# tangrizzly/Point-of-Interest-Recommendation

Measured on AMD Instinct MI355X. Metric: check-in sequences/sec training (Distance2Pre) + all-POI top-K eval users/sec, higher is better.
Workload: dtype f32 (forward pass: int8 x 5 fixed point + f64 gates); 1 GPU; synthetic gowalla-shape: 100000 POIs, 50000 users, seq<=50, dim=128, 200 distance bins; one step = one Distance2Pre training epoch over all users; batch_rule=capped sum, cap 64, parallelism=user-shard x1, per-epoch delta all-reduce, table_storage=f32

## Files before the change

### point-of-interest-recommendation_amd/csrc/abi.hip

```cpp
#include "../../include/poi_hip.h"
#include "poi_kernels.h"

#include <math.h>
#include <stdarg.h>
#include <stdio.h>
#include <stdlib.h>
#include <string.h>
#include <string>
#include <utility>
#include <vector>

namespace {
thread_local std::string g_err;
}

struct DevBuf {
  void* p = nullptr;
  size_t bytes = 0;
};

struct poi_ctx {
  int device = 0;
  int num_cu = 0;
  int wg_per_cu = 2;
  std::string err;
  DevBuf ws, slab, te_ws, hslab, zrow;
  DevBuf ex_ws, ex_slab, ex_glt, ex_gdi;
  int engine = 0;
  float batch_cap = 1.0f;
  int wgrad_rounds = 2;
  int head_rounds = 3;
  int score_variant = -1;
  DevBuf g_lt, mult_lt, nseq_lt, g_di, mult_di, nseq_di;
  DevBuf g_wd, mult_wd, nseq_wd, ca_ws, ca_slab, ca_scr, ca2;
  int carnn_fast = 1;
  hipEvent_t ev_hr0 = nullptr, ev_hr1 = nullptr;
  int hot_early = 1;
  hipStream_t side2 = nullptr; hipEvent_t ev_h0 = nullptr, ev_h1 = nullptr, ev_h2 = nullptr, ev_h3 = nullptr;
  int hybrid = 1, hyb_min = 1150, hyb_max = 2300, hyb_force = 0;
  hipStream_t side = nullptr; hipEvent_t ev_slots = nullptr, ev_sorted = nullptr, ev_bwd = nullptr, ev_fin = nullptr, ev_start = nullptr, ev_pack = nullptr;
  DevBuf seg_s, seg_e;
  DevBuf xc;
  DevBuf pmark;
  int ppoi = 1;
  int hot_bins = 1;
  int early_bins = 1;
  int early_min = 1024;
  DevBuf kc_dev;
  DevBuf ptab, iota;
  int iota_n = -1;
  int fwd_tab = 1;
  int bintab_min = 1280;
  int one_path = 1;
// ... 208 lines not shown
  ++c->te_ws_gen;
  const int n_dist = spatial ? P->n_dist : -1;
  const int D = P->dim, NBP = poi::te_nbp(n_dist);
  A.lt = P->lt; A.di = P->di; A.ui = P->ui; A.wh = P->wh; A.bi = P->bi; A.vs = P->vs; A.bs = P->bs; A.wd = P->wd; A.lw = P->lw;
  A.n_item = P->n_item; A.n_dist = n_dist; A.dim = D;
  A.spatial = spatial ? 1 : 0; A.xw = spatial ? 2 * D : D;
  A.lt_f16 = is_f16(c, P->lt);
  A.bintab = (poi::te_bintab(D, spatial, n_dist) && (predict || n >= c->bintab_min)) ? 1 : 0;
  A.rec32 = (D >= 256 || (D == 128 && c->engine == 3)) ? 1 : 0;
  A.rec_split = c->rec_split ? 1 : 0;
  A.head_split = (c->rec_split && A.spatial && (P->n_dist + 1 > 256 || (c->head3 && !predict))) ? 1 : 0;
  A.efuse = (c->efuse && A.head_split && !predict && P->n_dist + 1 <= 256 && D == 128) ? 1 : 0;
  A.rec1 = (!A.rec32 && n <= c->rec1_max) ? 1 : 0;
  A.hyb = (c->hybrid && c->side2 && !predict && !A.rec32 && D == 128 && c->xfwd && poi::te_xfwd_supported(D) && c->rec_split && n >= c->hyb_min && n <= c->hyb_max && n <= TE_HYB_NMAX && n > 1) ? 1 : 0;
  A.hyb_force = c->hyb_force;
  if (A.hyb) A.rec1 = 0;
  A.ppoi = (A.bintab && !predict && c->ppoi) ? 1 : 0;
  A.off = T->off; A.p = T->p; A.q = T->q; A.dp = T->dp; A.dq = T->dq; A.len_max = T->len_max;
  A.uidx = uidx; A.n_seq = n; A.predict = predict ? 1 : 0;
  if (const char* e = getenv("POI_TE_DBG")) A.dbg = atoi(e);
  A.dl = poi::dense_layout(D, A.xw, n_dist + 1);
  const size_t Tcap = (size_t)n * (size_t)(predict ? T->max_len : (T->max_len > 1 ? T->max_len - 1 : 1)) + 192;
  const size_t pk = (size_t)30 * D * D + (size_t)3 * NBP * D + 128;
  const bool sorted = !predict;
  const size_t Ncap = sorted ? 3 * (Tcap + (size_t)n) : 0;
  const size_t n_hot = Ncap / (TE_COLD_MAX + 1) + 2, n_chunk = Ncap / TE_HOT_CHUNK + n_hot + 2;
  const size_t sfl = sorted ? Tcap + n_chunk * D + Tcap * (size_t)NBP + (size_t)((n <= c->rec1_max || n <= c->hyb_max) ? n : (n + 15) / 16) * 3 * D + (size_t)2 * ((n + 255) / 256) + 128 : 0;
  const int Rrows = P->n_item + 1 + n_dist + 1;
  const bool listed = sorted && (size_t)Rrows > 4 * Ncap;
  const size_t sin = sorted ? 7 * Ncap + (listed ? Ncap : 0) + (size_t)RS_HIST_INTS + RS_MAXBIN + 16 + 4 * n_hot + 3 * n_chunk + 64 : 0;
// ... 55 lines not shown
  A.pVsT = (float4*)take((size_t)NBP * D * 3 / 2); A.pVs = (float4*)take((size_t)NBP * D * 3 / 2);
  A.pWhT16 = (float4*)take((size_t)9 * D * D / 2); A.pWhc16 = (float4*)take((size_t)3 * D * D / 2); A.pWhzr16 = (float4*)take((size_t)3 * D * D);
  if (A.hyb) { A.pWhc1 = (float4*)take((size_t)D * D); A.pWhzr1 = (float4*)take((size_t)2 * D * D); } else { A.pWhc1 = A.pWhc16; A.pWhzr1 = A.pWhzr16; }
  if (A.bintab) {
    A.ztab = take(NBt * 3 * D); A.dsum = take(NBt * 3 * D); A.dgd = take(NBt * D);
    if (sorted) { A.dpart = take(n_dchunk * (size_t)(3 * D)); A.dpart2 = take(n_dsuper * (size_t)(3 * D)); }
  }
  if (A.ppoi) { A.S = take(Tcap * (size_t)(3 * D)); A.pfirst = take(n_prange * (size_t)(3 * D)); A.plast = take(n_prange * (size_t)(3 * D)); }
  if (sorted) {
    A.gcoef = take(Tcap); A.hot_part = take(n_chunk * D); A.DL = take(Tcap * (size_t)NBP);
    A.bi_part = take((size_t)((A.rec1 || A.hyb) ? n : (n + 15) / 16) * 3 * D); A.fin_part = take((size_t)2 * ((n + 255) / 256) + 8);
  }
  int* ip = (int*)f;
  auto itake = [&](size_t cnt) { int* r = ip; ip += (cnt + 3) & ~(size_t)3; return r; };
  A.hyb_dev = itake(8);
  A.soff = itake(n + 1); A.row_src = itake(Tcap); A.row_t = itake(Tcap); A.row_p = itake(Tcap); A.row_dp = itake(Tcap); A.row_ab = itake(Tcap); A.row_pq = (int2*)itake(2 * Tcap);
  if (sorted) {
    int bits = 1; while ((1 << bits) <= R) ++bits;
    A.key_bits = bits;
    A.keys0 = itake(Ncap); A.keys1 = itake(Ncap); A.vals0 = itake(Ncap); A.vals1 = itake(Ncap);
    A.code = itake(Ncap); A.slot_seq = itake(Ncap); A.ent = itake(Ncap);
    A.hist = itake(RS_HIST_INTS + RS_MAXBIN);
    A.cnt = itake(8);
    A.urow = listed ? itake(Ncap) : nullptr;
    A.hot_rows = (int4*)itake(4 * n_hot); A.hot_chunks = (int2*)itake(2 * n_chunk); A.hot_nf = itake(n_chunk);
    A.seg_start = (int*)c->seg_s.p; A.seg_end = (int*)c->seg_e.p;
    A.dch0 = itake(NBt + 8); A.dhot = itake(NBt + 16); A.dcc0 = itake(NBt + 8);
    if (A.ppoi) {
      A.urow_p = itake(Tcap); A.pblk = itake(2 * 1024); A.dxe = itake(Tcap); A.dxs = itake(Tcap); A.dstart = itake(Tcap + 4);
      A.pmark = (int*)c->pmark.p;
// ... 1519 lines not shown
}

int poi_ctx_set_exact_forward(poi_ctx* c, int on, int per_sequence_max) {
  if (!c || on < 0 || on > 1) return fail(c, POI_EINVAL, "poi_ctx_set_exact_forward: on must be 0 or 1");
  c->xfwd = on;
  if (per_sequence_max >= 0) c->xrec1_max = per_sequence_max;
  drop_graphs(c);
  return POI_OK;
}

int poi_ctx_set_option(poi_ctx* c, const char* name, int value) {
  if (!c || !name) return fail(c, POI_EINVAL, "poi_ctx_set_option: null argument");
  struct Opt { const char* name; int* p; int lo, hi; };
  const Opt opts[] = {{"forward_table_compact", &c->xcomp, 0, 1}, {"forward_table_compact_min", &c->xcomp_min, 0, 1 << 30}, {"head_split", &c->head3, 0, 1},
                      {"early_bins", &c->early_bins, 0, 1}, {"hot_bins", &c->hot_bins, 0, 1}, {"hybrid", &c->hybrid, 0, 1}, {"hybrid_min", &c->hyb_min, 0, 1 << 30}, {"hybrid_max", &c->hyb_max, 0, 1 << 30}, {"hybrid_force", &c->hyb_force, 0, 1 << 30},
                      {"cell_grid", &c->cell_grid, 0, 1 << 30}, {"vbpr_grid", &c->vbpr_grid, 0, 1 << 30}, {"session_tile_min", &c->sess_tile_min, 1, 1 << 30},
                      {"near_split_max", &c->near_split_max, 0, 1 << 30}, {"near_grid", &c->near_grid, 0, NEAR_SPLIT_LIMIT},
                      {"rank_grid", &c->rank_grid, 0, 1 << 30}};
  for (const Opt& o : opts)
    if (!strcmp(name, o.name)) {
      if (value < o.lo || value > o.hi) return fail(c, POI_EINVAL, "poi_ctx_set_option: %s must be in [%d, %d] (got %d)", name, o.lo, o.hi, value);
      *o.p = value;
      drop_graphs(c);
      return POI_OK;
    }
  return fail(c, POI_EINVAL, "poi_ctx_set_option: unknown option '%s'", name);
}

int poi_ctx_set_small_launch(poi_ctx* c, int max_sequences) {
  if (!c || max_sequences < 0) return fail(c, POI_EINVAL, "poi_ctx_set_small_launch: max_sequences must be >= 0");
// ... 163 lines not shown
```

### point-of-interest-recommendation_amd/csrc/poi_common.h

```cpp
#pragma once
#include <hip/hip_runtime.h>
#include <mutex>
#include <hip/hip_fp16.h>
#include <stdint.h>

#define POI_WAVE 64
#define POI_BLOCK 256
#define POI_NWAVE (POI_BLOCK / POI_WAVE)

namespace poi {

__device__ __forceinline__ int lane_id() { return threadIdx.x & 63; }
__device__ __forceinline__ int wave_id() { return threadIdx.x >> 6; }

template <int CTRL>
__device__ __forceinline__ float dpp_f(float v) {
  return __int_as_float(__builtin_amdgcn_update_dpp(0, __float_as_int(v), CTRL, 0xF, 0xF, false));
}
__device__ __forceinline__ float readlane_f(float v, int l) {
  return __int_as_float(__builtin_amdgcn_readlane(__float_as_int(v), l));
}

__device__ __forceinline__ float wave_sum(float v) {
  v += dpp_f<0xB1>(v);
  v += dpp_f<0x4E>(v);
  v += dpp_f<0x141>(v);
  v += dpp_f<0x140>(v);
  return (readlane_f(v, 0) + readlane_f(v, 16)) + (readlane_f(v, 32) + readlane_f(v, 48));
// ... 222 lines not shown
struct DeviceOnce {
  std::mutex mu;
  bool done[64] = {};
  template <class F> hipError_t run(F&& f) {
    int dev = 0;
    hipError_t e = hipGetDevice(&dev);
    if (e != hipSuccess) return e;
    if (dev < 0 || dev >= 64) return hipErrorInvalidDevice;
    std::lock_guard<std::mutex> lock(mu);
    if (done[dev]) return hipSuccess;
    e = f();
    if (e == hipSuccess) done[dev] = true;
    return e;
  }
};
}
```

### point-of-interest-recommendation_amd/csrc/poi_kernels.h

```cpp
#pragma once
#include <hip/hip_runtime.h>
#include <stddef.h>
#include <stdint.h>

#include <string>
#include <vector>

namespace poi {

struct Timing {
  struct Rec { std::string name; hipEvent_t a, b; };
  bool on = false;
  int period = 1; unsigned long count = 0; bool active = true;
  void tick() { active = period <= 1 || (count++ % (unsigned long)period) == 0; }
  std::vector<Rec> recs;
  size_t limit = 32768;
  void begin(const char* name, hipStream_t st) {
    if (!on || !active || recs.size() >= limit) { open_ = false; return; }
    Rec r; r.name = name;
    if (hipEventCreate(&r.a) != hipSuccess || hipEventCreate(&r.b) != hipSuccess) { open_ = false; return; }
    (void)hipEventRecord(r.a, st);
    recs.push_back(r); open_ = true;
  }
  void end(hipStream_t st) { if (open_) { (void)hipEventRecord(recs.back().b, st); open_ = false; } }
// ... 89 lines not shown
  float* ptab; const int* iota; int fwd_tab; float* uiP;
  float4* pUiP3;
  float* uiT;
  float4 *pWhT16, *pWhc16, *pWhzr16;
  int rec_split;
  int head_split;
  int rec1;
  float* slab;
  int n_slab, n_head, n_kc;
  hipStream_t side; hipEvent_t ev_slots, ev_sorted;
  hipEvent_t ev_start, ev_pack;
  hipEvent_t ev_bwd, ev_fin;
  int hot_early; hipEvent_t ev_hr0, ev_hr1;
  int hyb, hyb_force; int* hyb_dev; float4 *pWhc1, *pWhzr1;
  hipStream_t side2; hipEvent_t ev_h0, ev_h1, ev_h2, ev_h3;
  float *bi_part, *fin_part;
  float* hslab; int hstride;
  DenseLayout dl;
  int *mult_lt, *nseq_lt, *mult_di, *nseq_di;
  float *hts, *sts; const int* out_row;
  int key_bits;
  int *keys0, *keys1, *vals0, *vals1;
  int *code, *slot_seq;
  int *ent;
  int *seg_start, *seg_end;
  int *hist;
  int *cnt;
  int *urow;
  int4* hot_rows;
  int2* hot_chunks;
// ... 458 lines not shown
```

### point-of-interest-recommendation_amd/csrc/te_xfwd.hip

```cpp
#include "poi_common.h"
#include "poi_kernels.h"

#include <stdio.h>
#include <type_traits>

namespace poi {

typedef int i32x4 __attribute__((ext_vector_type(4)));
typedef int i32x16 __attribute__((ext_vector_type(16)));

#define XS 5
#define XQB (8 * XS - 2)

__device__ __forceinline__ void x_lds_barrier() {
  asm volatile("s_waitcnt lgkmcnt(0)" ::: "memory");
  __builtin_amdgcn_s_barrier();
  asm volatile("" ::: "memory");
}
__device__ __forceinline__ double x_pow2(int e) { return __longlong_as_double((long long)(1023 + e) << 52); }
__device__ __forceinline__ int x_exponent(float m) { return (int)((__float_as_uint(m) >> 23) & 255u) - 126; }

__device__ __forceinline__ void x_digits(double t, unsigned& lo, unsigned& hi) {
  const unsigned long long b = (unsigned long long)__double_as_longlong(t + 0x1.8p52) + 0x8080808080ull;
  lo = (unsigned)b ^ 0x80808080u;
// ... 248 lines not shown
#else
#define XP_INIT
#define XP(i)
#define XP_END
#endif
struct XG12 { double v[12]; };

template <int D, bool FT, bool PRED = false>
__global__ __launch_bounds__(D * 4) void te_rec_fwdx_kernel(TeArgs A) {
  constexpr int KB = D / 64, NW = D / 16, SR = 3, SL = XS - SR, LDP = D + 16, PSZ = 16 * LDP;
  static_assert(D <= 128 && D % 64 == 0, "te_rec_fwdx: resident digit fragments and x_combine's int32 merge are sized for K <= 128");
  extern __shared__ __align__(16) unsigned char xlds[];
  unsigned char* Hq = xlds;
  unsigned char* RHq = Hq + XS * PSZ;
  uint4* Bl = reinterpret_cast<uint4*>(RHq + XS * PSZ) + (size_t)wave_id() * (3 * KB * SL * 64);
  __shared__ int s_r0[16], s_ns[16];
  __shared__ double s_t64[64];
  __shared__ __align__(16) double s_cn[3 * D];
  const int lane = lane_id(), w = wave_id(), tid = threadIdx.x, i = lane & 15;
  const int u0 = 16 * w + 4 * (lane >> 4);
  const int tile = blockIdx.x;
  const int k_lo = (!PRED && A.hyb) ? A.hyb_dev[0] : 0;
  if (k_lo + tile * 16 >= A.n_seq) return;
  if (tid < 16) {
    const int k = k_lo + tile * 16 + tid;
    int r0 = 0, ns = 0;
    if (k < A.n_seq) { r0 = A.soff[k]; ns = A.soff[k + 1] - r0; }
    s_r0[tid] = r0; s_ns[tid] = ns;
  }
  if (tid >= 64 && tid < 128) s_t64[tid - 64] = exp2((double)(tid - 64) * (1.0 / 64.0));
  for (int e = tid; e < 3 * D; e += blockDim.x) s_cn[e] = A.xWhS[e] * 0x1p-8;
  for (int e = tid; e < 2 * XS * PSZ / 4; e += blockDim.x) reinterpret_cast<unsigned*>(xlds)[e] = 0u;
  i32x4 bw[3][KB][SR];
#pragma unroll
  for (int gt = 0; gt < 3; ++gt) {
    const int nt = gt * NW + w;
#pragma unroll
    for (int kb = 0; kb < KB; ++kb)
#pragma unroll
      for (int s = 0; s < XS; ++s) {
        const uint4 v = A.xWh8[((size_t)(nt * KB + kb) * XS + s) * 64 + lane];
        if (s < SR) bw[gt][kb][s] = __builtin_bit_cast(i32x4, v);
        else Bl[((gt * KB + kb) * SL + (s - SR)) * 64 + lane] = v;
      }
  }
  __syncthreads();
  int ns_max = 0;
  for (int q = 0; q < 16; ++q) ns_max = max(ns_max, s_ns[q]);
  const int rowb = s_r0[i], nsr = s_ns[i];
  const int Tsp = A.soff[A.n_seq];
  const double h_init = (A.xflag && *A.xflag == A.xlaunch) ? __longlong_as_double(0x7FF8000000000000ll) : 0.0;
  double hcur[4] = {h_init, h_init, h_init, h_init};
  XG12 gc;
  struct XG4 { double v[4]; };
  auto load3 = [&](XG12& o, const double* __restrict__ rowp) {
#pragma unroll
    for (int g = 0; g < 3; ++g) {
      const XG4 q = *reinterpret_cast<const XG4*>(rowp + g * D + u0);
#pragma unroll
      for (int r = 0; r < 4; ++r) o.v[4 * g + r] = q.v[r];
    }
  };
  XP_INIT

  const unsigned char* hrow = Hq + i * LDP + 16 * (lane >> 4);
  const unsigned char* rrow = RHq + i * LDP + 16 * (lane >> 4);
  auto put_digits = [&](unsigned char* plane0, const double (&v)[4]) {
    unsigned lo[4], hi[4];
#pragma unroll
    for (int r = 0; r < 4; ++r) x_digits38(v[r], lo[r], hi[r]);
    unsigned* at = reinterpret_cast<unsigned*>(plane0 + i * LDP + u0);
    at[0] = x_gather_byte(hi[0], hi[1], hi[2], hi[3], 0);
#pragma unroll
    for (int s = 1; s < XS; ++s) at[s * (PSZ / 4)] = x_gather_byte(lo[0], lo[1], lo[2], lo[3], XS - 1 - s);
  };
  auto mma = [&](auto& acc, const unsigned char* __restrict__ h0, const int gt0, auto ng) {
    constexpr int NG = decltype(ng)::value;
#pragma unroll
    for (int g = 0; g < NG; ++g)
// ... 71 lines not shown
    auto fetch = [&](int t, XG12& n) { load3(n, A.gx + (size_t)(t < nsr ? rowb + t : Tsp) * 3 * D); };
    XG12 nx;
    fetch(0, gc);
    for (int t = 0; t < ns_max; ++t) {
      fetch(t + 1, nx);
      compute(t);
#pragma unroll
      for (int q = 0; q < 12; ++q) {
        asm volatile("" : "+v"(nx.v[q]));
        gc.v[q] = nx.v[q];
      }
    }
  } else {
    int rp = 0, rz = 0;
    const int* __restrict__ xrow = A.xcomp ? A.row_pc : A.row_p;
    auto ids = [&](int t) { const int rr = t < nsr ? rowb + t : Tsp; rp = xrow[rr]; rz = A.spatial ? A.row_dp[rr] : 0; };
    auto rows = [&](XG12& pp, XG12& zz) {
      const int p1 = (int)min((unsigned)rp, (unsigned)A.n_item), z1 = A.spatial ? (int)min((unsigned)rz, (unsigned)A.n_dist) : 0;
      load3(pp, A.ptabx + (size_t)p1 * 3 * D);
      load3(zz, A.ztabx + (size_t)z1 * 3 * D);
    };
    XG12 pn, zn;
    ids(0); rows(pn, zn);
#pragma unroll
    for (int q = 0; q < 12; ++q) gc.v[q] = pn.v[q] + zn.v[q];
    ids(1);
    for (int t = 0; t < ns_max; ++t) {
      rows(pn, zn);
      ids(t + 2);
      compute(t);
#pragma unroll
      for (int q = 0; q < 12; ++q) {
        asm volatile("" : "+v"(pn.v[q]), "+v"(zn.v[q]));
        gc.v[q] = pn.v[q] + zn.v[q];
      }
    }
  }
  if constexpr (PRED) {
    const int k = tile * 16 + i;
    if (k < A.n_seq)
      *reinterpret_cast<float4*>(A.hts + (size_t)(A.out_row ? A.out_row[k] : k) * D + u0) = make_float4((float)hcur[0], (float)hcur[1], (float)hcur[2], (float)hcur[3]);
  }
  XP_END
}

template <int CTRL>
__device__ __forceinline__ double x_dpp(double v) {
  const long long b = __double_as_longlong(v);
  const int lo = __builtin_amdgcn_update_dpp(0, (int)b, CTRL, 0xF, 0xF, false), hi = __builtin_amdgcn_update_dpp(0, (int)(b >> 32), CTRL, 0xF, 0xF, false);
  return __longlong_as_double(((long long)hi << 32) | (unsigned)lo);
}
template <int N> __device__ __forceinline__ double x_group_sum(double v) {
  v += x_dpp<0xB1>(v);
  v += x_dpp<0x4E>(v);
  v += x_dpp<0x141>(v);
  if (N >= 16) v += x_dpp<0x140>(v);
// ... 262 lines not shown
size_t te_xfwd_lds(int D) {
  const int KB = D / 64, NW = D / 16, SL = XS - 3;
  return (size_t)2 * XS * 16 * (D + 16) + (size_t)NW * 3 * KB * SL * 64 * 16;
}

size_t te_xfrag_bytes(int rows, int K) { return (size_t)rows * K * XS; }

template <int D> struct XRec {
  static constexpr bool F64 = D > 128;
  static size_t lds() { return F64 ? sizeof(double) * 2 * D * 16 : te_xfwd_lds(D <= 128 ? D : 128); }
  static dim3 block() { return dim3(F64 ? D * 2 : D * 4); }
  template <bool FT, bool PRED> static const void* fn() {
    if constexpr (F64) return reinterpret_cast<const void*>(&te_rec_fwdd_kernel<D, FT, PRED>);
    else return reinterpret_cast<const void*>(&te_rec_fwdx_kernel<D, FT, PRED>);
  }
  template <bool FT, bool PRED> static void launch(const TeArgs& A, hipStream_t st) {
    const dim3 grid((A.n_seq + 15) / 16);
    if constexpr (F64) hipLaunchKernelGGL((te_rec_fwdd_kernel<D, FT, PRED>), grid, block(), lds(), st, A);
    else hipLaunchKernelGGL((te_rec_fwdx_kernel<D, FT, PRED>), grid, block(), lds(), st, A);
  }
};

template <int D>
static hipError_t te_xfwd_t(const TeArgs& A, int num_cu, hipStream_t st, Timing* tm, int phase) {
  static DeviceOnce once;
  {
    const hipError_t oe = once.run([&]() -> hipError_t {
      const void* fns[5] = {XRec<D>::template fn<false, false>(), XRec<D>::template fn<true, false>(), XRec<D>::template fn<false, true>(), XRec<D>::template fn<true, true>(),
                            reinterpret_cast<const void*>(&te_gemmx_kernel<D>)};
      for (const void* f : fns) {
        const hipError_t e = hipFuncSetAttribute(f, hipFuncAttributeMaxDynamicSharedMemorySize, 152 * 1024);
        if (e != hipSuccess) return e;
      }
      return hipSuccess;
// ... 58 lines not shown
      for (int i = 0; i < 8; ++i) fprintf(stderr, " %s %.1f%%;", nm[i], 100.0 * (double)h[w][i] / (double)tot);
      fprintf(stderr, "\n");
    }
    unsigned long long z[8][10] = {};
    (void)hipMemcpyToSymbol(HIP_SYMBOL(g_xprof), z, sizeof(z));
  } } dump_at_exit;
#endif
  if (A.predict) {
    if constexpr (!XRec<D>::F64) {
      if (A.xrec1) {
        if (A.xft) hipLaunchKernelGGL((te_rec_fwd1x_kernel<D, true, true>), dim3(min(n, num_cu * (D <= 64 ? 3 : 1))), dim3(4 * D), 0, st, A);
        else hipLaunchKernelGGL((te_rec_fwd1x_kernel<D, true, false>), dim3(min(n, num_cu * (D <= 64 ? 3 : 1))), dim3(4 * D), 0, st, A);
        return hipGetLastError();
      }
    }
    if (A.xft) XRec<D>::template launch<true, true>(A, st);
    else XRec<D>::template launch<false, true>(A, st);
    return hipGetLastError();
  }
  tm->begin("te_rec_fwd", st);
  bool done = false;
  if constexpr (!XRec<D>::F64) {
    if (A.hyb) {
      if (hipEventRecord(A.ev_h0, st) != hipSuccess || hipStreamWaitEvent(A.side2, A.ev_h0, 0) != hipSuccess) return hipGetLastError();
      if (A.xft) hipLaunchKernelGGL((te_rec_fwd1x_kernel<D, false, true>), dim3(min(n, num_cu)), dim3(4 * D), 0, A.side2, A);
      else hipLaunchKernelGGL((te_rec_fwd1x_kernel<D, false, false>), dim3(min(n, num_cu)), dim3(4 * D), 0, A.side2, A);
      if (hipEventRecord(A.ev_h1, A.side2) != hipSuccess) return hipGetLastError();
      if (A.xft) XRec<D>::template launch<true, false>(A, st);
      else XRec<D>::template launch<false, false>(A, st);
      if (hipStreamWaitEvent(st, A.ev_h1, 0) != hipSuccess) return hipGetLastError();
      done = true;
    } else
    if (A.xrec1) {
      if (A.xft) hipLaunchKernelGGL((te_rec_fwd1x_kernel<D, false, true>), dim3(min(n, num_cu * (D <= 64 ? 3 : 1))), dim3(4 * D), 0, st, A);
      else hipLaunchKernelGGL((te_rec_fwd1x_kernel<D, false, false>), dim3(min(n, num_cu * (D <= 64 ? 3 : 1))), dim3(4 * D), 0, st, A);
      done = true;
    }
  }
  if (!done) {
    if (A.xft) XRec<D>::template launch<true, false>(A, st);
    else XRec<D>::template launch<false, false>(A, st);
  }
  tm->end(st);
  return hipGetLastError();
}

hipError_t launch_te_xfwd(const TeArgs& A, int num_cu, hipStream_t st, Timing* tm, int phase) {
  if (A.dim == 64) return te_xfwd_t<64>(A, num_cu, st, tm, phase);
  if (A.dim == 128) return te_xfwd_t<128>(A, num_cu, st, tm, phase);
  if (A.dim == 256) return te_xfwd_t<256>(A, num_cu, st, tm, phase);
  return hipErrorInvalidValue;
}

}
```

### point-of-interest-recommendation_amd/csrc/tile_engine.hip

```cpp
#include "poi_common.h"
#include "poi_kernels.h"

#include <stdlib.h>
#include <stdio.h>

namespace poi {

typedef float f32x16 __attribute__((ext_vector_type(16)));

#define TE_BLOCK 256

__device__ __forceinline__ f32x16 mfma32(float a, float b, f32x16 c) {
  return __builtin_amdgcn_mfma_f32_32x32x2f32(a, b, c, 0, 0, 0);
}
__device__ __forceinline__ void lds_barrier() {
  asm volatile("s_waitcnt lgkmcnt(0)" ::: "memory");
  __builtin_amdgcn_s_barrier();
  asm volatile("" ::: "memory");
}
__device__ __forceinline__ float fast_tanh(float x) { return 1.0f - 2.0f * __builtin_amdgcn_rcpf(1.0f + __expf(2.0f * x)); }
__device__ __forceinline__ float fast_sigmoid(float x) { return __builtin_amdgcn_rcpf(1.0f + __expf(-x)); }
__device__ __forceinline__ int c_row(int r, int lane) { return (r & 3) + 8 * (r >> 2) + 4 * (lane >> 5); }

struct PackJob { const float* src; int sk, sn, K, N, K8, NT; float4* dst; int n16; };
// ... 475 lines not shown
#pragma unroll
      for (int o = 1; o < 16; o <<= 1) { const int t2 = __shfl_up(t, o, 64); t += lane >= o ? t2 : 0; }
      if (lane < 16) wtot[lane] = t;
    }
    __syncthreads();
    const int run = carry + inc - s + (w > 0 ? wtot[w - 1] : 0);
    if (base == 0) my_pre = run;
#pragma unroll
    for (int u = 0; u < 16; ++u) if (i0 + u < n) A.soff[i0 + u] = run + v[u];
    carry += wtot[15];
    __syncthreads();
  }
  if (tid == 1023) {
    const int total = carry;
    A.soff[n] = total;
    if (A.cnt) { A.cnt[0] = (A.spatial ? 3 : 2) * (total + n); A.cnt[1] = 0; A.cnt[2] = 0; A.cnt[3] = 0; A.cnt[4] = 0; A.cnt[5] = 0; }
  }
  if (A.hyb && n <= TE_HYB_NMAX) te_hybrid_choose(A, num_cu, my_max, my_pre, carry, s_hmax, s_hpre, s_hcost, s_harg, s_hlen);
}

#ifndef TE_SEQ_PER_WAVE
#define TE_SEQ_PER_WAVE 4
#endif
__device__ __forceinline__ void te_slots(const TeArgs& A, int k, int base, int L, int ns, int r0, int* pads_lt, int* pads_di) {
  const int lane = lane_id();
  const int nsec = A.spatial ? 3 : 2;
  const int S0 = nsec * (r0 + k), nslot = nsec * (ns + 1), sentinel = A.n_item + 1 + A.n_dist + 1;
  int plt = 0, pdi = 0;
  for (int e0 = 0; e0 < nslot; e0 += 64) {
    const int e = e0 + lane;
// ... 807 lines not shown
  sbz += __shfl_xor(sbz, 16, 64); sbr += __shfl_xor(sbr, 16, 64); sbc += __shfl_xor(sbc, 16, 64);
  sbz += __shfl_xor(sbz, 32, 64); sbr += __shfl_xor(sbr, 32, 64); sbc += __shfl_xor(sbc, 32, 64);
  if (lane < 16) {
    float* bp = A.bi_part + (size_t)tile * 3 * D;
    bp[col] = sbz; bp[D + col] = sbr; bp[2 * D + col] = sbc;
  }
}

template <int D>
__global__ __launch_bounds__(D * 4) void te_rec_bwd16t_kernel(TeArgs A) {
  extern __shared__ __align__(16) float lds[];
  constexpr int KG2 = D / 32, LHA = D + 8, LHB = 2 * D + 8;
  unsigned short* Acs = reinterpret_cast<unsigned short*>(lds);
  unsigned short* Azrs = Acs + 3 * 16 * LHA;
  uint4* B3 = reinterpret_cast<uint4*>(Azrs + 3 * 16 * LHB) + (size_t)wave_id() * 3 * KG2 * 64;
  __shared__ int s_r0[16], s_ns[16];
  const int lane = lane_id(), w = wave_id(), tid = threadIdx.x;
  const int sq = lane & 15, u0 = 16 * w + 4 * (lane >> 4);
  const int tile = blockIdx.x;
  const int k_lo = A.hyb ? A.hyb_dev[2] : 0;
  if (k_lo + tile * 16 >= A.n_seq) return;
  if (tid < 16) {
    const int k = k_lo + tile * 16 + tid;
    int r0 = 0, ns = 0;
    if (k < A.n_seq) { r0 = A.soff[k]; ns = A.soff[k + 1] - r0; }
    s_r0[tid] = r0; s_ns[tid] = ns;
  }
  lds_barrier();
  int ns_max = 0;
  for (int i = 0; i < 16; ++i) ns_max = max(ns_max, s_ns[i]);
  const int rowb = s_r0[sq], nsr = s_ns[sq];
  uint4 bcb[KG2][2], bzrb[2 * KG2][2];
  const uint4 *cc3 = B3 + lane, *czr3 = B3 + KG2 * 64 + lane;
  load_bfrag3<KG2>(bcb, B3, A.pWhc16, w);
  load_bfrag3<2 * KG2>(bzrb, B3 + KG2 * 64, A.pWhzr16, w);
  float dhn[4], sbz[4], sbr[4], sbc[4];
#pragma unroll
  for (int r = 0; r < 4; ++r) { dhn[r] = 0.f; sbz[r] = 0.f; sbr[r] = 0.f; sbc[r] = 0.f; }
  struct Ops { float4 z, r, c, h, d; };
  float fz[4], fr[4], fc[4], fh[4], fd[4];
  const int Tsp = A.soff[A.n_seq];
  auto fetch = [&](int t, Ops& X) {
    const bool on = t >= 0 && t < nsr;
    const size_t row = (size_t)(on ? rowb + t : Tsp);
    const float* g = A.G + row * 3 * D + u0;
    X.z = *reinterpret_cast<const float4*>(g); X.r = *reinterpret_cast<const float4*>(g + D); X.c = *reinterpret_cast<const float4*>(g + 2 * D);
    X.h = *reinterpret_cast<const float4*>(A.H + (on && t > 0 ? row - 1 : (size_t)Tsp) * D + u0);
    X.d = *reinterpret_cast<const float4*>(A.DH + row * D + u0);
  };
  auto take = [&](Ops& X, int t) {
    asm volatile("" : "+v"(X.z.x), "+v"(X.z.y), "+v"(X.z.z), "+v"(X.z.w), "+v"(X.r.x), "+v"(X.r.y), "+v"(X.r.z), "+v"(X.r.w), "+v"(X.c.x), "+v"(X.c.y), "+v"(X.c.z), "+v"(X.c.w));
    asm volatile("" : "+v"(X.h.x), "+v"(X.h.y), "+v"(X.h.z), "+v"(X.h.w), "+v"(X.d.x), "+v"(X.d.y), "+v"(X.d.z), "+v"(X.d.w));
    const bool on = t >= 0 && t < nsr, onh = on && t > 0;
    fz[0] = on ? X.z.x : 0.f; fz[1] = on ? X.z.y : 0.f; fz[2] = on ? X.z.z : 0.f; fz[3] = on ? X.z.w : 0.f;
    fr[0] = on ? X.r.x : 0.f; fr[1] = on ? X.r.y : 0.f; fr[2] = on ? X.r.z : 0.f; fr[3] = on ? X.r.w : 0.f;
    fc[0] = on ? X.c.x : 0.f; fc[1] = on ? X.c.y : 0.f; fc[2] = on ? X.c.z : 0.f; fc[3] = on ? X.c.w : 0.f;
// ... 51 lines not shown
  fetch(t - 1, B1);
  for (; t >= 1; t -= 2) {
    fetch(t - 2, B0); compute(t); take(B1, t - 1);
    fetch(t - 3, B1); compute(t - 1); take(B0, t - 2);
  }
  if (t == 0) compute(0);
#pragma unroll
  for (int r = 0; r < 4; ++r)
#pragma unroll
    for (int o = 1; o < 16; o <<= 1) { sbz[r] += __shfl_xor(sbz[r], o, 64); sbr[r] += __shfl_xor(sbr[r], o, 64); sbc[r] += __shfl_xor(sbc[r], o, 64); }
  if (sq == 0) {
    float* bp = A.bi_part + (size_t)(k_lo + tile) * 3 * D + u0;
    *reinterpret_cast<float4*>(bp) = make_float4(sbz[0], sbz[1], sbz[2], sbz[3]);
    *reinterpret_cast<float4*>(bp + D) = make_float4(sbr[0], sbr[1], sbr[2], sbr[3]);
    *reinterpret_cast<float4*>(bp + 2 * D) = make_float4(sbc[0], sbc[1], sbc[2], sbc[3]);
  }
}

template <int N> __device__ __forceinline__ float group_sum(float v) {
  v += dpp_f<0xB1>(v);
  v += dpp_f<0x4E>(v);
  v += dpp_f<0x141>(v);
  if (N >= 16) v += dpp_f<0x140>(v);
  return v;
}
typedef float f32x2 __attribute__((ext_vector_type(2)));
template <int L>
__device__ __forceinline__ void dot4_reg_lds(const f32x2 (&w)[2][L], const float* __restrict__ x, float (&a)[4]) {
  f32x2 p0 = {a[0], a[1]}, p1 = {a[2], a[3]};
#pragma unroll
// ... 1941 lines not shown
    NtArgs P{nullptr, 0, A.lt, A.di, A.row_p, nullptr, D, A.ui, D, A.G, 3 * D, A.bi, A.soff + n, 3 * D, D, nullptr, nullptr};
    if constexpr (D >= 128) hipLaunchKernelGGL((te_gemm_ntk_kernel<true, true, D, D, 3 * D, D, 3 * D, false, F16>), grid, block, 0, st, P);
    else hipLaunchKernelGGL((te_gemm_nt_kernel<true, true, F16>), grid, block, 0, st, P);
  }
}

template <int D>
static void te_launch_ax(const TeArgs& A, int num_cu, hipStream_t st) {
  if (A.lt_f16) te_launch_ax_t<D, true>(A, num_cu, st);
  else te_launch_ax_t<D, false>(A, num_cu, st);
}

template <int D>
static hipError_t te_one_t(TeArgs& A, float alpha, float lambda, int l_cap, hipStream_t st, Timing* tm) {
  if constexpr (D > 128) { return hipErrorInvalidValue; } else {
  PackJobs J; te_pack_jobs(A, J, true);
  const int n_ax = 3 * D / 16, n_pk = 8, NB = A.n_dist + 1;
  tm->begin("te_prep", st);
  hipLaunchKernelGGL(te_one_in_kernel<D>, dim3(n_ax + 1 + n_pk * J.n), dim3(TE_BLOCK), 0, st, A, J, n_ax, n_pk);
  tm->end(st);
  if (A.xfwd) {
    hipError_t xe = A.xrec1 ? hipSuccess : launch_te_xfwd(A, 64, st, tm, 2);
    if (xe == hipSuccess) xe = launch_te_xfwd(A, 64, st, tm, 1);
    if (xe != hipSuccess) return xe;
  } else {
  tm->begin("te_rec_fwd", st);
  hipLaunchKernelGGL((te_rec_fwd1_kernel<D, false>), dim3(1), dim3(4 * D), 0, st, A);
  tm->end(st);
  }
  tm->begin("te_head", st);
// ... 99 lines not shown
  tm->begin("te_head", st);
  if (A.spatial) {
    hipError_t e = te_head_dispatch<D>(A, 0, A.n_head, st);
    if (e != hipSuccess) return e;
  } else {
    hipLaunchKernelGGL(te_bpr_head_kernel<D>, dim3(num_cu * 8), dim3(TE_BLOCK), 0, st, A);
  }
  tm->end(st);
  if (A.hot_early) {
    if (hipEventRecord(A.ev_hr0, st) != hipSuccess || hipStreamWaitEvent(A.side, A.ev_hr0, 0) != hipSuccess) return hipGetLastError();
    const long sp = tm->span_begin("te_hot_early", A.side);
    hipError_t he = launch_te_hot_reduce(A, num_cu, A.side); if (he != hipSuccess) return he;
    tm->span_end(sp, A.side);
    if (hipEventRecord(A.ev_hr1, A.side) != hipSuccess) return hipGetLastError();
  }
  tm->begin("te_rec_bwd", st);
  if constexpr (D >= 128) {
    if (A.rec32 && A.rec_split) hipLaunchKernelGGL((te_rec_bwd32_kernel<D, D / 32, true>), dim3((n + 31) / 32), dim3(D * 2), sizeof(short) * 3 * 32 * (3 * D + 16), st, A);
    else if (A.rec32) hipLaunchKernelGGL((te_rec_bwd32_kernel<D, D / 32>), dim3((n + 31) / 32), dim3(D * 2), sizeof(float) * (32 * (D + 4) + 32 * (2 * D + 4)), st, A);
  }
  if constexpr (D <= 128) {
    if (!A.rec32) {
      if (A.hyb) {
        const bool serial = (A.dbg & 8192) != 0;
        hipStream_t s2 = serial ? st : A.side2;
        if (!serial && (hipEventRecord(A.ev_h2, st) != hipSuccess || hipStreamWaitEvent(A.side2, A.ev_h2, 0) != hipSuccess)) return hipGetLastError();
        hipLaunchKernelGGL(te_rec_bwd1_kernel<D>, dim3(min(n, num_cu)), dim3(4 * D), 0, s2, A);
        if (!serial && hipEventRecord(A.ev_h3, A.side2) != hipSuccess) return hipGetLastError();
        hipLaunchKernelGGL((te_rec_bwd16t_kernel<D>), dim3((n + 15) / 16), dim3(D * 4), sizeof(short) * (3 * 16 * (3 * D + 16) + 3 * D * D), st, A);
        if (!serial && hipStreamWaitEvent(st, A.ev_h3, 0) != hipSuccess) return hipGetLastError();
      } else
      if (A.rec1) hipLaunchKernelGGL(te_rec_bwd1_kernel<D>, dim3(min(n, num_cu * (D <= 64 ? 4 : 1))), dim3(4 * D), 0, st, A);
      else if (A.rec_split && !(A.dbg & 128)) hipLaunchKernelGGL((te_rec_bwd16t_kernel<D>), dim3((n + 15) / 16), dim3(D * 4), sizeof(short) * (3 * 16 * (3 * D + 16) + 3 * D * D), st, A);
      else if (A.rec_split) hipLaunchKernelGGL((te_rec_bwd16_kernel<D, true>), dim3((n + 15) / 16), dim3(D * 4), sizeof(short) * (3 * 16 * (3 * D + 16) + 3 * D * D), st, A);
      else hipLaunchKernelGGL((te_rec_bwd16_kernel<D, false>), dim3((n + 15) / 16), dim3(D * 4), sizeof(float) * (16 * (D + 4) + 16 * (2 * D + 4)), st, A);
    }
  }
  tm->end(st);
  const int n_fin = (n + TE_BLOCK - 1) / TE_BLOCK, n_out = 3 * D + (A.spatial ? A.n_dist + 4 : 0);
  auto finalize = [&](hipStream_t s) {
    tm->begin("te_finalize", s);
    hipLaunchKernelGGL(te_finalize_kernel, dim3(n_fin), dim3(TE_BLOCK), 0, s, A);
    hipLaunchKernelGGL(te_parts_kernel, dim3((n_out + POI_NWAVE - 1) / POI_NWAVE), dim3(TE_BLOCK), 0, s, A, A.rec1 ? n : A.rec32 ? (n + 31) / 32 : (n + 15) / 16, n_fin);
    tm->end(s);
  };
  if (A.side) {
    if (hipEventRecord(A.ev_bwd, st) != hipSuccess || hipStreamWaitEvent(A.side, A.ev_bwd, 0) != hipSuccess) return hipGetLastError();
    finalize(A.side);
// ... 146 lines not shown
```

Baseline: 7.620 million sequences/s.

## Make recurrent forward/backward tile kernels persistent with atomic tile queue

Turns the per-tile recurrent forward (xfwd) and backward (bwd16t) kernels into persistent kernels. The grid is capped at CU count times occupancy, and each workgroup pulls its next 16-sequence tile from an atomic counter that is reset in the prefix kernel. This amortises the per-block setup (weight fragment loads into registers and LDS, constant tables) across many tiles and balances work across variable-length tiles. The cost is an atomic per tile, an extra barrier per iteration, and LDS zeroing moved inside the loop.

```diff
diff --git a/point-of-interest-recommendation_amd/csrc/abi.hip b/point-of-interest-recommendation_amd/csrc/abi.hip
--- a/point-of-interest-recommendation_amd/csrc/abi.hip
+++ b/point-of-interest-recommendation_amd/csrc/abi.hip
@@ -37,6 +37,7 @@
   hipEvent_t ev_hr0 = nullptr, ev_hr1 = nullptr;
   int hot_early = 1;
   hipStream_t side2 = nullptr; hipEvent_t ev_h0 = nullptr, ev_h1 = nullptr, ev_h2 = nullptr, ev_h3 = nullptr;
+  int rec_persistent = 1, rec_grid = 0;
   int hybrid = 1, hyb_min = 1150, hyb_max = 2300, hyb_force = 0;
   hipStream_t side = nullptr; hipEvent_t ev_slots = nullptr, ev_sorted = nullptr, ev_bwd = nullptr, ev_fin = nullptr, ev_start = nullptr, ev_pack = nullptr;
   DevBuf seg_s, seg_e;
@@ -275,6 +276,7 @@
   A.rec1 = (!A.rec32 && n <= c->rec1_max) ? 1 : 0;
   A.hyb = (c->hybrid && c->side2 && !predict && !A.rec32 && D == 128 && c->xfwd && poi::te_xfwd_supported(D) && c->rec_split && n >= c->hyb_min && n <= c->hyb_max && n <= TE_HYB_NMAX && n > 1) ? 1 : 0;
   A.hyb_force = c->hyb_force;
+  A.rec_pers = c->rec_persistent; A.rec_grid = c->rec_grid; A.rec_cu = c->num_cu;
   if (A.hyb) A.rec1 = 0;
   A.ppoi = (A.bintab && !predict && c->ppoi) ? 1 : 0;
   A.off = T->off; A.p = T->p; A.q = T->q; A.dp = T->dp; A.dq = T->dq; A.len_max = T->len_max;
@@ -360,6 +362,7 @@
   int* ip = (int*)f;
   auto itake = [&](size_t cnt) { int* r = ip; ip += (cnt + 3) & ~(size_t)3; return r; };
   A.hyb_dev = itake(8);
+  A.rec_q = A.hyb_dev + 4;
   A.soff = itake(n + 1); A.row_src = itake(Tcap); A.row_t = itake(Tcap); A.row_p = itake(Tcap); A.row_dp = itake(Tcap); A.row_ab = itake(Tcap); A.row_pq = (int2*)itake(2 * Tcap);
   if (sorted) {
     int bits = 1; while ((1 << bits) <= R) ++bits;
@@ -1909,6 +1912,7 @@
   struct Opt { const char* name; int* p; int lo, hi; };
   const Opt opts[] = {{"forward_table_compact", &c->xcomp, 0, 1}, {"forward_table_compact_min", &c->xcomp_min, 0, 1 << 30}, {"head_split", &c->head3, 0, 1},
                       {"early_bins", &c->early_bins, 0, 1}, {"hot_bins", &c->hot_bins, 0, 1}, {"hybrid", &c->hybrid, 0, 1}, {"hybrid_min", &c->hyb_min, 0, 1 << 30}, {"hybrid_max", &c->hyb_max, 0, 1 << 30}, {"hybrid_force", &c->hyb_force, 0, 1 << 30},
+                      {"rec_persistent", &c->rec_persistent, 0, 1}, {"rec_grid", &c->rec_grid, 0, 1 << 30},
                       {"cell_grid", &c->cell_grid, 0, 1 << 30}, {"vbpr_grid", &c->vbpr_grid, 0, 1 << 30}, {"session_tile_min", &c->sess_tile_min, 1, 1 << 30},
                       {"near_split_max", &c->near_split_max, 0, 1 << 30}, {"near_grid", &c->near_grid, 0, NEAR_SPLIT_LIMIT},
                       {"rank_grid", &c->rank_grid, 0, 1 << 30}};
diff --git a/point-of-interest-recommendation_amd/csrc/poi_common.h b/point-of-interest-recommendation_amd/csrc/poi_common.h
--- a/point-of-interest-recommendation_amd/csrc/poi_common.h
+++ b/point-of-interest-recommendation_amd/csrc/poi_common.h
@@ -12,6 +12,11 @@
 
 __device__ __forceinline__ int lane_id() { return threadIdx.x & 63; }
 __device__ __forceinline__ int wave_id() { return threadIdx.x >> 6; }
+__device__ __forceinline__ int lane_id_again() {
+  int l;
+  asm volatile("v_mbcnt_lo_u32_b32 %0, -1, 0\n\tv_mbcnt_hi_u32_b32 %0, -1, %0" : "=v"(l));
+  return l;
+}
 
 template <int CTRL>
 __device__ __forceinline__ float dpp_f(float v) {
@@ -264,4 +269,23 @@
     return e;
   }
 };
-}
+struct DeviceOccupancy {
+  std::mutex mu;
+  int per_cu[64] = {};
+  hipError_t get(const void* fn, int block, size_t lds, int* out) {
+    int dev = 0;
+    hipError_t e = hipGetDevice(&dev);
+    if (e != hipSuccess) return e;
+    if (dev < 0 || dev >= 64) return hipErrorInvalidDevice;
+    std::lock_guard<std::mutex> lock(mu);
+    if (!per_cu[dev]) {
+      int nb = 0;
+      e = hipOccupancyMaxActiveBlocksPerMultiprocessor(&nb, fn, block, lds);
+      if (e != hipSuccess) return e;
+      per_cu[dev] = nb > 0 ? nb : 1;
+    }
+    *out = per_cu[dev];
+    return hipSuccess;
+  }
+};
+}
diff --git a/point-of-interest-recommendation_amd/csrc/poi_kernels.h b/point-of-interest-recommendation_amd/csrc/poi_kernels.h
--- a/point-of-interest-recommendation_amd/csrc/poi_kernels.h
+++ b/point-of-interest-recommendation_amd/csrc/poi_kernels.h
@@ -127,6 +127,7 @@
   int hot_early; hipEvent_t ev_hr0, ev_hr1;
   int hyb, hyb_force; int* hyb_dev; float4 *pWhc1, *pWhzr1;
   hipStream_t side2; hipEvent_t ev_h0, ev_h1, ev_h2, ev_h3;
+  int rec_pers, rec_grid, rec_cu; int* rec_q;
   float *bi_part, *fin_part;
   float* hslab; int hstride;
   DenseLayout dl;
diff --git a/point-of-interest-recommendation_amd/csrc/te_xfwd.hip b/point-of-interest-recommendation_amd/csrc/te_xfwd.hip
--- a/point-of-interest-recommendation_amd/csrc/te_xfwd.hip
+++ b/point-of-interest-recommendation_amd/csrc/te_xfwd.hip
@@ -286,23 +286,18 @@
   unsigned char* Hq = xlds;
   unsigned char* RHq = Hq + XS * PSZ;
   uint4* Bl = reinterpret_cast<uint4*>(RHq + XS * PSZ) + (size_t)wave_id() * (3 * KB * SL * 64);
-  __shared__ int s_r0[16], s_ns[16];
+  __shared__ int s_r0[16], s_ns[16], s_next;
   __shared__ double s_t64[64];
   __shared__ __align__(16) double s_cn[3 * D];
   const int lane = lane_id(), w = wave_id(), tid = threadIdx.x, i = lane & 15;
   const int u0 = 16 * w + 4 * (lane >> 4);
-  const int tile = blockIdx.x;
   const int k_lo = (!PRED && A.hyb) ? A.hyb_dev[0] : 0;
-  if (k_lo + tile * 16 >= A.n_seq) return;
-  if (tid < 16) {
-    const int k = k_lo + tile * 16 + tid;
-    int r0 = 0, ns = 0;
-    if (k < A.n_seq) { r0 = A.soff[k]; ns = A.soff[k + 1] - r0; }
-    s_r0[tid] = r0; s_ns[tid] = ns;
-  }
+  const int n_tile = (A.n_seq - k_lo + 15) / 16;
+  int tile = blockIdx.x;
+  if (tile >= n_tile) return;
+  const int ws = __builtin_amdgcn_readfirstlane(w);
   if (tid >= 64 && tid < 128) s_t64[tid - 64] = exp2((double)(tid - 64) * (1.0 / 64.0));
   for (int e = tid; e < 3 * D; e += blockDim.x) s_cn[e] = A.xWhS[e] * 0x1p-8;
-  for (int e = tid; e < 2 * XS * PSZ / 4; e += blockDim.x) reinterpret_cast<unsigned*>(xlds)[e] = 0u;
   i32x4 bw[3][KB][SR];
 #pragma unroll
   for (int gt = 0; gt < 3; ++gt) {
@@ -316,12 +311,28 @@
         else Bl[((gt * KB + kb) * SL + (s - SR)) * 64 + lane] = v;
       }
   }
+  const int Tsp = A.soff[A.n_seq];
+  const double h_init = (A.xflag && *A.xflag == A.xlaunch) ? __longlong_as_double(0x7FF8000000000000ll) : 0.0;
+  auto spare = [&]() -> int {
+    if constexpr (FT && PRED) { int v; asm volatile("v_mov_b32 %0, %1" : "=v"(v) : "s"(Tsp)); return v; }
+    else return Tsp;
+  };
+  XP_INIT
+  for (;;) {
+  const int ln = lane_id_again();
+  if (ws == 0 && ln < 16) {
+    const int k = k_lo + tile * 16 + ln;
+    int r0 = 0, ns = 0;
+    if (k < A.n_seq) { r0 = A.soff[k]; ns = A.soff[k + 1] - r0; }
+    s_r0[ln] = r0; s_ns[ln] = ns;
+  }
+  if (A.rec_pers && ws == 1 && ln == 0) s_next = (int)gridDim.x + atomicAdd(A.rec_q, 1);
+  for (int e = 64 * ws + ln; e < 2 * XS * PSZ / 4; e += 4 * D) reinterpret_cast<unsigned*>(xlds)[e] = 0u;
   __syncthreads();
   int ns_max = 0;
   for (int q = 0; q < 16; ++q) ns_max = max(ns_max, s_ns[q]);
-  const int rowb = s_r0[i], nsr = s_ns[i];
-  const int Tsp = A.soff[A.n_seq];
-  const double h_init = (A.xflag && *A.xflag == A.xlaunch) ? __longlong_as_double(0x7FF8000000000000ll) : 0.0;
+  ns_max = __builtin_amdgcn_readfirstlane(ns_max);
+  const int rowb = s_r0[ln & 15], nsr = s_ns[ln & 15];
   double hcur[4] = {h_init, h_init, h_init, h_init};
   XG12 gc;
   struct XG4 { double v[4]; };
@@ -333,8 +344,6 @@
       for (int r = 0; r < 4; ++r) o.v[4 * g + r] = q.v[r];
     }
   };
-  XP_INIT
-
   const unsigned char* hrow = Hq + i * LDP + 16 * (lane >> 4);
   const unsigned char* rrow = RHq + i * LDP + 16 * (lane >> 4);
   auto put_digits = [&](unsigned char* plane0, const double (&v)[4]) {
@@ -436,7 +445,7 @@
   } else {
     int rp = 0, rz = 0;
     const int* __restrict__ xrow = A.xcomp ? A.row_pc : A.row_p;
-    auto ids = [&](int t) { const int rr = t < nsr ? rowb + t : Tsp; rp = xrow[rr]; rz = A.spatial ? A.row_dp[rr] : 0; };
+    auto ids = [&](int t) { const int rr = t < nsr ? rowb + t : spare(); rp = xrow[rr]; rz = A.spatial ? A.row_dp[rr] : 0; };
     auto rows = [&](XG12& pp, XG12& zz) {
       const int p1 = (int)min((unsigned)rp, (unsigned)A.n_item), z1 = A.spatial ? (int)min((unsigned)rz, (unsigned)A.n_dist) : 0;
       load3(pp, A.ptabx + (size_t)p1 * 3 * D);
@@ -459,9 +468,14 @@
     }
   }
   if constexpr (PRED) {
-    const int k = tile * 16 + i;
+    const int l2 = lane_id_again(), k = tile * 16 + (l2 & 15);
     if (k < A.n_seq)
-      *reinterpret_cast<float4*>(A.hts + (size_t)(A.out_row ? A.out_row[k] : k) * D + u0) = make_float4((float)hcur[0], (float)hcur[1], (float)hcur[2], (float)hcur[3]);
+      *reinterpret_cast<float4*>(A.hts + (size_t)(A.out_row ? A.out_row[k] : k) * D + 16 * ws + 4 * (l2 >> 4)) = make_float4((float)hcur[0], (float)hcur[1], (float)hcur[2], (float)hcur[3]);
+  }
+  if (!A.rec_pers) break;
+  tile = __builtin_amdgcn_readfirstlane(s_next);
+  x_lds_barrier();
+  if (tile >= n_tile) break;
   }
   XP_END
 }
@@ -754,10 +768,21 @@
     if constexpr (F64) return reinterpret_cast<const void*>(&te_rec_fwdd_kernel<D, FT, PRED>);
     else return reinterpret_cast<const void*>(&te_rec_fwdx_kernel<D, FT, PRED>);
   }
-  template <bool FT, bool PRED> static void launch(const TeArgs& A, hipStream_t st) {
-    const dim3 grid((A.n_seq + 15) / 16);
-    if constexpr (F64) hipLaunchKernelGGL((te_rec_fwdd_kernel<D, FT, PRED>), grid, block(), lds(), st, A);
-    else hipLaunchKernelGGL((te_rec_fwdx_kernel<D, FT, PRED>), grid, block(), lds(), st, A);
+  template <bool FT, bool PRED> static hipError_t launch(const TeArgs& A, hipStream_t st) {
+    int tiles = (A.n_seq + 15) / 16;
+    if constexpr (F64) hipLaunchKernelGGL((te_rec_fwdd_kernel<D, FT, PRED>), dim3(tiles), block(), lds(), st, A);
+    else {
+      if (A.rec_pers) {
+        static DeviceOccupancy occ;
+        int per_cu = 1;
+        const hipError_t e = occ.get(fn<FT, PRED>(), (int)block().x, lds(), &per_cu);
+        if (e != hipSuccess) return e;
+        tiles = min(tiles, max(A.rec_cu, 1) * per_cu);
+        if (A.rec_grid > 0) tiles = min(tiles, A.rec_grid);
+      }
+      hipLaunchKernelGGL((te_rec_fwdx_kernel<D, FT, PRED>), dim3(tiles), block(), lds(), st, A);
+    }
+    return hipSuccess;
   }
 };
 
@@ -846,8 +871,7 @@
         return hipGetLastError();
       }
     }
-    if (A.xft) XRec<D>::template launch<true, true>(A, st);
-    else XRec<D>::template launch<false, true>(A, st);
+    { const hipError_t le = A.xft ? XRec<D>::template launch<true, true>(A, st) : XRec<D>::template launch<false, true>(A, st); if (le != hipSuccess) return le; }
     return hipGetLastError();
   }
   tm->begin("te_rec_fwd", st);
@@ -858,8 +882,7 @@
       if (A.xft) hipLaunchKernelGGL((te_rec_fwd1x_kernel<D, false, true>), dim3(min(n, num_cu)), dim3(4 * D), 0, A.side2, A);
       else hipLaunchKernelGGL((te_rec_fwd1x_kernel<D, false, false>), dim3(min(n, num_cu)), dim3(4 * D), 0, A.side2, A);
       if (hipEventRecord(A.ev_h1, A.side2) != hipSuccess) return hipGetLastError();
-      if (A.xft) XRec<D>::template launch<true, false>(A, st);
-      else XRec<D>::template launch<false, false>(A, st);
+      { const hipError_t le = A.xft ? XRec<D>::template launch<true, false>(A, st) : XRec<D>::template launch<false, false>(A, st); if (le != hipSuccess) return le; }
       if (hipStreamWaitEvent(st, A.ev_h1, 0) != hipSuccess) return hipGetLastError();
       done = true;
     } else
@@ -870,8 +893,7 @@
     }
   }
   if (!done) {
-    if (A.xft) XRec<D>::template launch<true, false>(A, st);
-    else XRec<D>::template launch<false, false>(A, st);
+    { const hipError_t le = A.xft ? XRec<D>::template launch<true, false>(A, st) : XRec<D>::template launch<false, false>(A, st); if (le != hipSuccess) return le; }
   }
   tm->end(st);
   return hipGetLastError();
diff --git a/point-of-interest-recommendation_amd/csrc/tile_engine.hip b/point-of-interest-recommendation_amd/csrc/tile_engine.hip
--- a/point-of-interest-recommendation_amd/csrc/tile_engine.hip
+++ b/point-of-interest-recommendation_amd/csrc/tile_engine.hip
@@ -513,6 +513,7 @@
   if (tid == 1023) {
     const int total = carry;
     A.soff[n] = total;
+    A.rec_q[0] = 0; A.rec_q[1] = 0;
     if (A.cnt) { A.cnt[0] = (A.spatial ? 3 : 2) * (total + n); A.cnt[1] = 0; A.cnt[2] = 0; A.cnt[3] = 0; A.cnt[4] = 0; A.cnt[5] = 0; }
   }
   if (A.hyb && n <= TE_HYB_NMAX) te_hybrid_choose(A, num_cu, my_max, my_pre, carry, s_hmax, s_hpre, s_hcost, s_harg, s_hlen);
@@ -1350,32 +1351,37 @@
   unsigned short* Acs = reinterpret_cast<unsigned short*>(lds);
   unsigned short* Azrs = Acs + 3 * 16 * LHA;
   uint4* B3 = reinterpret_cast<uint4*>(Azrs + 3 * 16 * LHB) + (size_t)wave_id() * 3 * KG2 * 64;
-  __shared__ int s_r0[16], s_ns[16];
+  __shared__ int s_r0[16], s_ns[16], s_next;
   const int lane = lane_id(), w = wave_id(), tid = threadIdx.x;
   const int sq = lane & 15, u0 = 16 * w + 4 * (lane >> 4);
-  const int tile = blockIdx.x;
   const int k_lo = A.hyb ? A.hyb_dev[2] : 0;
-  if (k_lo + tile * 16 >= A.n_seq) return;
-  if (tid < 16) {
-    const int k = k_lo + tile * 16 + tid;
-    int r0 = 0, ns = 0;
-    if (k < A.n_seq) { r0 = A.soff[k]; ns = A.soff[k + 1] - r0; }
-    s_r0[tid] = r0; s_ns[tid] = ns;
-  }
-  lds_barrier();
-  int ns_max = 0;
-  for (int i = 0; i < 16; ++i) ns_max = max(ns_max, s_ns[i]);
-  const int rowb = s_r0[sq], nsr = s_ns[sq];
+  const int n_tile = (A.n_seq - k_lo + 15) / 16;
+  int tile = blockIdx.x;
+  if (tile >= n_tile) return;
+  const int ws = __builtin_amdgcn_readfirstlane(w);
   uint4 bcb[KG2][2], bzrb[2 * KG2][2];
   const uint4 *cc3 = B3 + lane, *czr3 = B3 + KG2 * 64 + lane;
   load_bfrag3<KG2>(bcb, B3, A.pWhc16, w);
   load_bfrag3<2 * KG2>(bzrb, B3 + KG2 * 64, A.pWhzr16, w);
+  const int Tsp = A.soff[A.n_seq];
+  for (;;) {
+  const int ln = lane_id_again();
+  if (ws == 0 && ln < 16) {
+    const int k = k_lo + tile * 16 + ln;
+    int r0 = 0, ns = 0;
+    if (k < A.n_seq) { r0 = A.soff[k]; ns = A.soff[k + 1] - r0; }
+    s_r0[ln] = r0; s_ns[ln] = ns;
+  }
+  if (A.rec_pers && ws == 1 && ln == 0) s_next = (int)gridDim.x + atomicAdd(A.rec_q + 1, 1);
+  lds_barrier();
+  int ns_max = 0;
+  for (int i = 0; i < 16; ++i) ns_max = max(ns_max, s_ns[i]);
+  const int rowb = s_r0[ln & 15], nsr = s_ns[ln & 15];
   float dhn[4], sbz[4], sbr[4], sbc[4];
 #pragma unroll
   for (int r = 0; r < 4; ++r) { dhn[r] = 0.f; sbz[r] = 0.f; sbr[r] = 0.f; sbc[r] = 0.f; }
   struct Ops { float4 z, r, c, h, d; };
   float fz[4], fr[4], fc[4], fh[4], fd[4];
-  const int Tsp = A.soff[A.n_seq];
   auto fetch = [&](int t, Ops& X) {
     const bool on = t >= 0 && t < nsr;
     const size_t row = (size_t)(on ? rowb + t : Tsp);
@@ -1457,6 +1463,11 @@
     *reinterpret_cast<float4*>(bp) = make_float4(sbz[0], sbz[1], sbz[2], sbz[3]);
     *reinterpret_cast<float4*>(bp + D) = make_float4(sbr[0], sbr[1], sbr[2], sbr[3]);
     *reinterpret_cast<float4*>(bp + 2 * D) = make_float4(sbc[0], sbc[1], sbc[2], sbc[3]);
+  }
+  if (!A.rec_pers) break;
+  tile = __builtin_amdgcn_readfirstlane(s_next);
+  lds_barrier();
+  if (tile >= n_tile) break;
   }
 }
 
@@ -3428,6 +3439,7 @@
 template <int D>
 static hipError_t te_one_t(TeArgs& A, float alpha, float lambda, int l_cap, hipStream_t st, Timing* tm) {
   if constexpr (D > 128) { return hipErrorInvalidValue; } else {
+  A.rec_pers = 0;
   PackJobs J; te_pack_jobs(A, J, true);
   const int n_ax = 3 * D / 16, n_pk = 8, NB = A.n_dist + 1;
   tm->begin("te_prep", st);
@@ -3557,6 +3569,18 @@
     tm->span_end(sp, A.side);
     if (hipEventRecord(A.ev_hr1, A.side) != hipSuccess) return hipGetLastError();
   }
+  int g16t = (n + 15) / 16;
+  const size_t lds16t = sizeof(short) * (3 * 16 * (3 * D + 16) + 3 * D * D);
+  if constexpr (D <= 128) {
+    if (A.rec_pers && !A.rec32 && !A.rec1 && A.rec_split) {
+      static DeviceOccupancy occ;
+      int per_cu = 1;
+      const hipError_t oe = occ.get(reinterpret_cast<const void*>(&te_rec_bwd16t_kernel<D>), D * 4, lds16t, &per_cu);
+      if (oe != hipSuccess) return oe;
+      g16t = min(g16t, max(A.rec_cu, 1) * per_cu);
+      if (A.rec_grid > 0) g16t = min(g16t, A.rec_grid);
+    }
+  }
   tm->begin("te_rec_bwd", st);
   if constexpr (D >= 128) {
     if (A.rec32 && A.rec_split) hipLaunchKernelGGL((te_rec_bwd32_kernel<D, D / 32, true>), dim3((n + 31) / 32), dim3(D * 2), sizeof(short) * 3 * 32 * (3 * D + 16), st, A);
@@ -3570,11 +3594,12 @@
         if (!serial && (hipEventRecord(A.ev_h2, st) != hipSuccess || hipStreamWaitEvent(A.side2, A.ev_h2, 0) != hipSuccess)) return hipGetLastError();
         hipLaunchKernelGGL(te_rec_bwd1_kernel<D>, dim3(min(n, num_cu)), dim3(4 * D), 0, s2, A);
         if (!serial && hipEventRecord(A.ev_h3, A.side2) != hipSuccess) return hipGetLastError();
-        hipLaunchKernelGGL((te_rec_bwd16t_kernel<D>), dim3((n + 15) / 16), dim3(D * 4), sizeof(short) * (3 * 16 * (3 * D + 16) + 3 * D * D), st, A);
+        if (g16t < (n + 15) / 16) hipLaunchKernelGGL((te_rec_bwd16t_kernel<D>), dim3(g16t), dim3(D * 4), lds16t, st, A);
+        else hipLaunchKernelGGL((te_rec_bwd16t_kernel<D>), dim3((n + 15) / 16), dim3(D * 4), sizeof(short) * (3 * 16 * (3 * D + 16) + 3 * D * D), st, A);
         if (!serial && hipStreamWaitEvent(st, A.ev_h3, 0) != hipSuccess) return hipGetLastError();
       } else
       if (A.rec1) hipLaunchKernelGGL(te_rec_bwd1_kernel<D>, dim3(min(n, num_cu * (D <= 64 ? 4 : 1))), dim3(4 * D), 0, st, A);
-      else if (A.rec_split && !(A.dbg & 128)) hipLaunchKernelGGL((te_rec_bwd16t_kernel<D>), dim3((n + 15) / 16), dim3(D * 4), sizeof(short) * (3 * 16 * (3 * D + 16) + 3 * D * D), st, A);
+      else if (A.rec_split && !(A.dbg & 128)) hipLaunchKernelGGL((te_rec_bwd16t_kernel<D>), dim3(g16t), dim3(D * 4), lds16t, st, A);
       else if (A.rec_split) hipLaunchKernelGGL((te_rec_bwd16_kernel<D, true>), dim3((n + 15) / 16), dim3(D * 4), sizeof(short) * (3 * 16 * (3 * D + 16) + 3 * D * D), st, A);
       else hipLaunchKernelGGL((te_rec_bwd16_kernel<D, false>), dim3((n + 15) / 16), dim3(D * 4), sizeof(float) * (16 * (D + 4) + 16 * (2 * D + 4)), st, A);
     }
```

Result: no change. 7.599 million sequences/s (-0.3%).
